# StractOrg/stract

Hardware: NVIDIA H100
Metric: webgraph_edges_per_sec_per_centrality_iter (higher is better)
Workload: dtype u8

## Files before the change

stract_b200/csrc/api_graph.cu:

```cuda
#include "graph.cuh"

#include <algorithm>
#include <vector>

namespace sb200 {
static thread_local char t_err[1024] = "";
std::atomic<uint64_t> g_launches{0};
thread_local cudaStream_t t_pool_stream = nullptr;
void set_error(const char* fmt, ...) {
  va_list ap; va_start(ap, fmt);
  vsnprintf(t_err, sizeof(t_err), fmt, ap);
  va_end(ap);
}
int hb_alloc_state(sb200_graph* g);
int hb_reset(sb200_graph* g);
int hb_step(sb200_graph* g, sb200_iter_stats* st);
int hb_step_launch(sb200_graph* g, bool with_barrier);
int hb_step_finish(sb200_graph* g, sb200_iter_stats* st);
int hb_barrier(sb200_graph* g);
__global__ void k_owned_flags(const uint32_t* __restrict__ inv, const uint32_t* __restrict__ sub, uint64_t N, uint32_t world, uint32_t rank,
                              uint8_t* owned, uint32_t* sub_out) {
  const uint64_t r = blockIdx.x * (uint64_t)blockDim.x + threadIdx.x;
  if (r >= N) return;
  const uint32_t v = inv[r];
  if (owned) owned[r] = (world <= 1 || ((v >> 5) % world) == rank) ? 1 : 0;
  if (sub_out) sub_out[r] = sub ? sub[v] : (world <= 1 ? 1u : 0xFFFFFFFFu >> (32 - world));
}
int hb_result(sb200_graph* g, uint64_t* id_lo, uint64_t* id_hi, double* cent, uint64_t cap, uint64_t* len);
int hb_registers(sb200_graph* g, uint64_t first, uint64_t count, uint8_t* out);
int hb_ranked(sb200_graph* g, int ties_desc, uint64_t* id_lo, uint64_t* id_hi, double* cent, uint64_t cap, uint64_t* len);
int hb_kahan(sb200_graph* g, uint64_t first, uint64_t count, double* sum, double* err);
}
using namespace sb200;

uint64_t sb200_graph::hbm_bytes() const {
  return id_lo.bytes() + id_hi.bytes() + perm.bytes() + inv.bytes() + row_ptr.bytes() + col.bytes() + fwd_ptr.bytes() +
         fwd_dst.bytes() + item_row.bytes() + item_start.bytes() + partial.bytes() + regs[0].bytes() + regs[1].bytes() +
         bm[0].bytes() + bm[1].bytes() + size_cache.bytes() + kahan_sum.bytes() + kahan_err.bytes() +
         frontier_list.bytes() + frontier_off.bytes() + cub_tmp.bytes() + counters.bytes() + sub_mask.bytes() + sync_page.bytes();
}

extern "C" {

const char* sb200_last_error(void) { return t_err; }
#ifndef SB200_EMU
const char* sb200_version(void) { return "stract_b200 0.1 (sm_90a)"; }
#else
const char* sb200_version(void) { return "stract_b200 0.1 CPU SIMT emulation (tests/emu, tests only)"; }
#endif
uint64_t sb200_kernel_launch_count(void) { return g_launches.load(); }

#define SB_ENTER(g)                                            \
  if (!(g)) SB_FAIL(SB200_EINVAL, "NULL graph handle");        \
  SB_CUDA(cudaSetDevice((g)->device))

int sb200_graph_create(const uint64_t* from_lo, const uint64_t* from_hi, const uint64_t* to_lo, const uint64_t* to_hi,
                       const uint64_t* rel_flags, uint64_t n_edges, uint64_t skipped_rel_mask, int device, int rank,
                       int world_size, sb200_graph** out) {
  if (!out) SB_FAIL(SB200_EINVAL, "out is NULL");
  *out = nullptr;
  if (world_size < 1 || world_size > 64 || rank < 0 || rank >= world_size)
    SB_FAIL(SB200_EINVAL, "bad rank/world_size %d/%d", rank, world_size);
  int ndev = 0;
  SB_CUDA(cudaGetDeviceCount(&ndev));
  if (device < 0 || device >= ndev) SB_FAIL(SB200_EINVAL, "device %d not in [0,%d)", device, ndev);
  SB_CUDA(cudaSetDevice(device));
  sb200_graph* g = new (std::nothrow) sb200_graph();
  if (!g) SB_FAIL(SB200_ENOMEM, "host allocation failed");
  g->device = device; g->rank = rank; g->world = world_size;
  int rc = SB200_OK;
  auto body = [&]() -> int {
    SB_CUDA(cudaStreamCreateWithFlags(&g->stream, cudaStreamNonBlocking));
    SB_CUDA(cudaEventCreate(&g->ev0)); SB_CUDA(cudaEventCreate(&g->ev1));
    SB_CUDA(cudaEventCreate(&g->ev_run0)); SB_CUDA(cudaEventCreate(&g->ev_run1));
    for (int f = 0; f < sb200_graph::F_COUNT; f++) { SB_CUDA(cudaEventCreate(&g->prof_ev[f][0])); SB_CUDA(cudaEventCreate(&g->prof_ev[f][1])); }
    {
      static bool pool_ready[64] = {false};
      if (device < 64 && !pool_ready[device]) {
        cudaMemPool_t pool; uint64_t keep = ~0ull;
        SB_CUDA(cudaDeviceGetDefaultMemPool(&pool, device));
        SB_CUDA(cudaMemPoolSetAttribute(pool, cudaMemPoolAttrReleaseThreshold, &keep));
        pool_ready[device] = true;
      }
      PoolScope scope(getenv("SB200_NO_POOL") ? nullptr : g->stream);
      SB_TRY(stage_graph(g, from_lo, from_hi, to_lo, to_hi, rel_flags, n_edges, skipped_rel_mask));
    }
    g->cub_tmp.release();
    {
      PoolScope scope((world_size == 1 && !getenv("SB200_NO_POOL")) ? g->stream : nullptr);
      SB_TRY(hb_alloc_state(g));
    }
    SB_TRY(hb_reset(g));
    return SB200_OK;
  };
  rc = body();
  if (rc != SB200_OK) { sb200_graph_destroy(g); return rc; }
  *out = g;
  return SB200_OK;
}

void sb200_graph_destroy(sb200_graph* g) {
  if (!g) return;
  cudaSetDevice(g->device);
  if (g->stream) cudaStreamSynchronize(g->stream);
  if (g->peers_ipc) for (int p = 0; p < g->n_peers; p++) for (int i = 0; i < 2; i++) {
    if (g->peer_regs[i][p]) cudaIpcCloseMemHandle(g->peer_regs[i][p]);
    if (g->peer_bm[i][p]) cudaIpcCloseMemHandle(g->peer_bm[i][p]);
  }
  if (g->peers_ipc) for (int p = 0; p < g->n_peers; p++) if (g->peer_sync[p]) cudaIpcCloseMemHandle(g->peer_sync[p]);
  if (g->l2_window_bytes) cudaCtxResetPersistingL2Cache();
  if (g->h_counters) cudaFreeHost(g->h_counters);
  if (g->ev0) cudaEventDestroy(g->ev0);
  if (g->ev1) cudaEventDestroy(g->ev1);
  if (g->side_stream) { cudaStreamSynchronize(g->side_stream); cudaStreamDestroy(g->side_stream); }
  if (g->ev_fork) cudaEventDestroy(g->ev_fork);
  if (g->ev_join) cudaEventDestroy(g->ev_join);
  for (int k = 0; k < 2; k++) if (g->side_prof[k]) cudaEventDestroy(g->side_prof[k]);
  if (g->ev_run0) cudaEventDestroy(g->ev_run0);
  if (g->ev_run1) cudaEventDestroy(g->ev_run1);
  for (int f = 0; f < sb200_graph::F_COUNT; f++) for (int k = 0; k < 2; k++) if (g->prof_ev[f][k]) cudaEventDestroy(g->prof_ev[f][k]);
  cudaStream_t s = g->stream;
  const int dev = g->device;
// ... 321 lines not shown
```

stract_b200/csrc/graph.cuh:

```cuda
#pragma once
#include "common.cuh"

namespace sb200 {
constexpr int MAX_PEERS = 15;
struct PeerOut { uint4* newr[MAX_PEERS]; uint32_t* bmc[MAX_PEERS]; const uint32_t* sub; int n; uint32_t world, rank; uint8_t prank[MAX_PEERS + 1]; };
constexpr int SYNC_SLOTS = 128;
struct SyncView { unsigned long long* local; unsigned long long* peer[MAX_PEERS]; int n; uint32_t world, rank; };
}

struct sb200_graph {
  int device = 0, rank = 0, world = 1;
  cudaStream_t stream = nullptr;
  cudaEvent_t ev0 = nullptr, ev1 = nullptr;
  uint64_t N = 0, E_in = 0, E_kept = 0, E_local = 0;
  uint64_t row_begin = 0, row_end = 0;
  uint64_t n_pos = 0;
  bool has_fwd = false;
  int reuse = 0;
  double stage_ms = 0;

  sb200::DevBuf<uint64_t> id_lo, id_hi;
  sb200::DevBuf<uint32_t> perm, inv;
  sb200::DevBuf<uint32_t> self_bm;
  sb200::DevBuf<uint32_t> row_ptr, col;
  uint32_t col_base = 0;
  sb200::DevBuf<uint32_t> fwd_ptr, fwd_dst;
  sb200::DevBuf<uint32_t> row_ranges_host_dummy;
  uint64_t range_begins[65] = {0};

  uint64_t warp_row_begin = 0, warp_row_end = 0;
  uint64_t quad_row_begin = 0, quad_row_end = 0;
  uint64_t n_items = 0;
  uint64_t n_multi_rows = 0;
  sb200::DevBuf<uint32_t> owned_items;
  uint64_t n_owned_items = 0;
  sb200::DevBuf<uint32_t> item_row, item_start;
  sb200::DevBuf<uint4> partial;
  uint64_t n_multi_items = 0;

  sb200::DevBuf<uint8_t> regs[2];
  sb200::DevBuf<uint32_t> bm[2];
  sb200::DevBuf<uint64_t> size_cache;
  sb200::DevBuf<double> kahan_sum, kahan_err;
  sb200::DevBuf<uint32_t> frontier_list, frontier_off;
  sb200::DevBuf<uint8_t> cub_tmp;
  sb200::DevBuf<unsigned long long> counters;
  unsigned long long* h_counters = nullptr;
  int cur = 0;
  int bcur = 0;
  uint32_t t = 0;
  bool has_changes = true;
  uint64_t n_changed_prev = 0, frontier_edges_prev = 0;
  bool exchange_pending = false;
  int n_peers = 0;
  bool p2p = false;
  bool peers_ipc = true;
  void* peer_regs[2][sb200::MAX_PEERS] = {{nullptr}};
  void* peer_bm[2][sb200::MAX_PEERS] = {{nullptr}};
  int peer_rank[sb200::MAX_PEERS] = {0};
  bool publish_all = false;
  sb200::DevBuf<uint32_t> sub_mask;
  uint64_t n_subscribed = 0;
  sb200::DevBuf<unsigned long long> sync_page;
  void* peer_sync[sb200::MAX_PEERS] = {nullptr};
  uint64_t sync_epoch = 0;
  bool step_in_flight = false, step_with_barrier = false;
  int step_mode = 0;
  double dense_frac = 0.35, push_div = 48.0;
  int force_mode = -1;
  uint64_t l2_window_bytes = 0;

  enum { F_PULL_WARP_DENSE, F_PULL_QUAD_DENSE, F_PULL_WARP_FRONT, F_PULL_QUAD_FRONT, F_PULL_MERGE, F_PUSH, F_FINALIZE, F_COUNT };
  bool profiling = false;
  uint64_t prof_launches[F_COUNT] = {0};
  double prof_ms[F_COUNT] = {0}, prof_bytes[F_COUNT] = {0};
  cudaEvent_t prof_ev[F_COUNT][2] = {{nullptr}};
  int sm_count = 0;
  int opt_side_ctas = -1, opt_owned_list = -1;
  cudaStream_t side_stream = nullptr;
  cudaEvent_t ev_fork = nullptr, ev_join = nullptr, side_prof[2] = {nullptr, nullptr};
  bool side_prof_used = false;
  int side_prof_family = 0;
  bool prof_used[F_COUNT] = {false};
  double prof_step_bytes[F_COUNT] = {0};
  uint64_t E_warp = 0, E_quad = 0;
  double own_frac = 1.0;
  cudaEvent_t ev_run0 = nullptr, ev_run1 = nullptr;
  float last_run_ms = 0;

  uint64_t hbm_bytes() const;
};

namespace sb200 {
constexpr int QUAD_MAX_DEG = 32;
constexpr int CHUNK_EDGES = 1024;

int build_fwd_csr(sb200_graph* g);
int stage_graph(sb200_graph* g, const uint64_t* from_lo, const uint64_t* from_hi, const uint64_t* to_lo,
                const uint64_t* to_hi, const uint64_t* rel, uint64_t n_edges, uint64_t mask);
}
```

stract_b200/csrc/hyperball.cu:

```cuda
#include <chrono>
#include "graph.cuh"
#include "../../include/sb200_hll_tables.h"

#ifndef SB200_EMU
#include <cub/cub.cuh>
#endif
#include <algorithm>
#include <cmath>
#include <cstdlib>

namespace sb200 {

struct HllTables {
  double raw[SB200_HLL_P5_LEN];
  double bias[SB200_HLL_P5_LEN];
  double lc[65];
};
__constant__ HllTables c_tab;
static bool g_tab_loaded[64] = {false};

int load_tables(int device) {
  if (device >= 0 && device < 64 && g_tab_loaded[device]) return SB200_OK;
  static HllTables h;
  for (int i = 0; i < SB200_HLL_P5_LEN; i++) { h.raw[i] = SB200_HLL_RAW_P5[i]; h.bias[i] = SB200_HLL_BIAS_P5[i]; }
// ... 218 lines not shown
  const unsigned ballA = __ballot_sync(0xffffffffu, ne_u4(accA, ownA)), ballB = __ballot_sync(0xffffffffu, ne_u4(accB, ownB));
  const bool chA = ((ballA >> (lane & ~3u)) & 0xFu) != 0u, chB = ((ballB >> (lane & ~3u)) & 0xFu) != 0u;
  if (liveA && (chA || bm_test(bm_prev, selfA))) newr[rowA * 4 + sub] = accA;
  if (liveA && chA && sub == 0) atomicOr(bm_cur + (selfA >> 5), 1u << (selfA & 31));
  if (liveB && (chB || bm_test(bm_prev, selfB))) newr[rowB * 4 + sub] = accB;
  if (liveB && chB && sub == 0) atomicOr(bm_cur + (selfB >> 5), 1u << (selfB & 31));
}

template <bool FRONTIER, bool LISTED>
__global__ void __launch_bounds__(256, 8) k_pull_warp(uint64_t n_items, uint64_t first_multi_free_item,
    const uint32_t* __restrict__ item_list, const uint32_t* __restrict__ item_row, const uint32_t* __restrict__ item_start, uint32_t warp_row_begin,
    const uint32_t* __restrict__ row_ptr, const uint32_t* __restrict__ col, uint32_t col_base,
    const uint4* __restrict__ oldr, uint4* __restrict__ newr, uint4* __restrict__ partial,
    const uint32_t* __restrict__ bm_prev, uint32_t* __restrict__ bm_cur, const PeerOut peers) {
  uint64_t item = (blockIdx.x * (uint64_t)blockDim.x + threadIdx.x) >> 5;
  if (item >= n_items) return;
  if (LISTED) item = item_list[item];
  const uint32_t lane = threadIdx.x & 31, sub = lane & 3, q = lane >> 2;
  const uint32_t row = item_row[item];
  if (!owned_row(peers, row)) return;
  const uint32_t chunk = (uint32_t)item - item_start[row - warp_row_begin];
  const uint32_t rs = row_ptr[row] - col_base, re = row_ptr[row + 1] - col_base;
  const uint32_t e0 = rs + chunk * (uint32_t)CHUNK_EDGES;
  const uint32_t e1 = min(e0 + (uint32_t)CHUNK_EDGES, re);
  uint4 acc = make_uint4(0, 0, 0, 0);
  uint32_t nxt = (e0 + lane < e1) ? ld_stream_u32(col + e0 + lane) : row;
  for (uint32_t base = e0; base < e1; base += 32) {
    uint32_t mine = nxt;
    nxt = (base + 32 + lane < e1) ? ld_stream_u32(col + base + 32 + lane) : row;
    if (FRONTIER) mine = bm_test(bm_prev, mine) ? mine : row;
    const uint32_t i0 = __shfl_sync(0xffffffffu, mine, q);
    const uint32_t i1 = __shfl_sync(0xffffffffu, mine, q + 8);
    const uint32_t i2 = __shfl_sync(0xffffffffu, mine, q + 16);
    const uint32_t i3 = __shfl_sync(0xffffffffu, mine, q + 24);
    const uint4 v0 = oldr[(uint64_t)i0 * 4 + sub];
    const uint4 v1 = oldr[(uint64_t)i1 * 4 + sub];
    const uint4 v2 = oldr[(uint64_t)i2 * 4 + sub];
    const uint4 v3 = oldr[(uint64_t)i3 * 4 + sub];
    acc = vmax_u8x16(vmax_u8x16(acc, v0), vmax_u8x16(vmax_u8x16(v1, v2), v3));
  }
#pragma unroll
  for (int off = 4; off < 32; off <<= 1) {
    uint4 o;
    o.x = __shfl_xor_sync(0xffffffffu, acc.x, off); o.y = __shfl_xor_sync(0xffffffffu, acc.y, off);
    o.z = __shfl_xor_sync(0xffffffffu, acc.z, off); o.w = __shfl_xor_sync(0xffffffffu, acc.w, off);
    acc = vmax_u8x16(acc, o);
  }
  if (item < first_multi_free_item) {
    if (q == 0) partial[item * 4 + sub] = acc;
    return;
  }
  const uint4 own = oldr[(uint64_t)row * 4 + sub];
  acc = vmax_u8x16(acc, own);
  const unsigned ball = __ballot_sync(0xffffffffu, ne_u4(acc, own));
  const bool changed = (ball & 0xFu) != 0u;
  if (q == 0) publish_row(newr, bm_cur, peers, row, sub, acc, changed || bm_test(bm_prev, row), changed);
}

__global__ void __launch_bounds__(256) k_pull_merge(uint64_t n_rows, const uint32_t* __restrict__ item_start,
    uint32_t warp_row_begin, const uint4* __restrict__ partial, const uint4* __restrict__ oldr,
    uint4* __restrict__ newr, const uint32_t* __restrict__ bm_prev, uint32_t* __restrict__ bm_cur, const PeerOut peers) {
  const uint64_t r = (blockIdx.x * (uint64_t)blockDim.x + threadIdx.x) >> 5;
  if (r >= n_rows) return;
  const uint32_t lane = threadIdx.x & 31, sub = lane & 3, q = lane >> 2;
  const uint32_t row = warp_row_begin + (uint32_t)r;
  if (!owned_row(peers, row)) return;
  const uint32_t i0 = item_start[r], i1 = item_start[r + 1];
  uint4 acc = make_uint4(0, 0, 0, 0);
  for (uint32_t it = i0 + q; it < i1; it += 8) acc = vmax_u8x16(acc, partial[(uint64_t)it * 4 + sub]);
#pragma unroll
  for (int off = 4; off < 32; off <<= 1) {
    uint4 o;
    o.x = __shfl_xor_sync(0xffffffffu, acc.x, off); o.y = __shfl_xor_sync(0xffffffffu, acc.y, off);
    o.z = __shfl_xor_sync(0xffffffffu, acc.z, off); o.w = __shfl_xor_sync(0xffffffffu, acc.w, off);
    acc = vmax_u8x16(acc, o);
  }
  const uint4 own = oldr[(uint64_t)row * 4 + sub];
  acc = vmax_u8x16(acc, own);
  const unsigned ball = __ballot_sync(0xffffffffu, ne_u4(acc, own));
  const bool changed = (ball & 0xFu) != 0u;
  if (q == 0) publish_row(newr, bm_cur, peers, row, sub, acc, changed || bm_test(bm_prev, row), changed);
}

__global__ void k_frontier_compact(const uint32_t* __restrict__ bm, uint64_t words, const uint32_t* __restrict__ fwd_ptr,
                                   uint32_t* list, uint32_t* outdeg, unsigned long long* counter,
                                   unsigned long long* slot_sum) {
  uint64_t w = blockIdx.x * (uint64_t)blockDim.x + threadIdx.x;
  if (w >= words) return;
  uint32_t m = bm[w];
  if (!m) return;
  unsigned long long pos = atomicAdd(counter, (unsigned long long)__popc(m));
  unsigned long long sum = 0;
  while (m) {
    int b = __ffs(m) - 1; m &= m - 1;
    uint32_t v = (uint32_t)(w * 32 + b);
    const uint32_t d = fwd_ptr[v + 1] - fwd_ptr[v];
    list[pos] = v; outdeg[pos] = d; pos++; sum += d;
  }
  if (slot_sum && sum) atomicAdd(slot_sum, sum);
}
__global__ void k_copy_stale(const uint32_t* __restrict__ list, uint64_t n, const uint4* __restrict__ oldr,
                             uint4* __restrict__ newr, uint32_t world, uint32_t rank) {
  uint64_t gt = blockIdx.x * (uint64_t)blockDim.x + threadIdx.x;
  uint64_t i = gt >> 2;
  if (i >= n) return;
  uint64_t v = list[i];
  if (world > 1 && ((v >> 5) % world) != rank) return;
  newr[v * 4 + (gt & 3)] = oldr[v * 4 + (gt & 3)];
}
__global__ void k_publish_rows(const uint32_t* __restrict__ bm_prev, const uint32_t* __restrict__ bm_cur, uint64_t n_rows,
                               const uint4* __restrict__ newr, const PeerOut peers) {
  const uint64_t gt = blockIdx.x * (uint64_t)blockDim.x + threadIdx.x;
  const uint64_t w = (gt >> 2) * peers.world + peers.rank;
  if (w * 32 >= n_rows) return;
  uint32_t m = __ldg(bm_prev + w) | __ldg(bm_cur + w);
  while (m) {
    const uint64_t row = w * 32 + (uint64_t)(__ffs(m) - 1);
    m &= m - 1;
    if (row >= n_rows) break;
    const uint4 v = newr[row * 4 + (gt & 3)];
    const uint32_t want = peers.sub ? __ldg(peers.sub + row) : 0xFFFFFFFFu;
    for (int p = 0; p < peers.n; p++) if ((want >> peers.prank[p]) & 1u) peers.newr[p][row * 4 + (gt & 3)] = v;
  }
}
__global__ void __launch_bounds__(256) k_push(const uint32_t* __restrict__ list, const uint32_t* __restrict__ off,
    uint32_t n_front, uint64_t n_slots, const uint32_t* __restrict__ fwd_ptr, const uint32_t* __restrict__ fwd_dst,
    const uint32_t* __restrict__ old32, uint32_t* new32, uint32_t* __restrict__ bm_cur) {
  const uint32_t lane = threadIdx.x & 31, l = lane & 15;
  const uint64_t hw = (blockIdx.x * (uint64_t)blockDim.x + threadIdx.x) >> 4;
  const uint64_t nhw = ((uint64_t)gridDim.x * blockDim.x) >> 4;
  for (uint64_t s = hw; s < ((n_slots + 1) & ~1ull); s += nhw) {
    bool changed = false;
    uint32_t v = 0;
    if (s < n_slots) {
      uint32_t lo = 0, hi = n_front;
      while (lo + 1 < hi) { uint32_t mid = (lo + hi) >> 1; if (off[mid] <= s) lo = mid; else hi = mid; }
      const uint32_t u = list[lo];
      v = fwd_dst[fwd_ptr[u] + (uint32_t)(s - off[lo])];
      const uint32_t mine = old32[(uint64_t)u * 16 + l];
      uint32_t* addr = new32 + (uint64_t)v * 16 + l;
      uint32_t cur = *addr;
      uint32_t m = bmax4_7bit(cur, mine);
      while (m != cur) {
        const uint32_t prev = atomicCAS(addr, cur, m);
        if (prev == cur) { changed = true; break; }
        cur = prev; m = bmax4_7bit(cur, mine);
      }
    }
    const unsigned ball = __ballot_sync(0xffffffffu, changed);
    const unsigned half = (lane < 16) ? (ball & 0xFFFFu) : (ball >> 16);
    if (half && l == 0) atomicOr(bm_cur + (v >> 5), 1u << (v & 31));
  }
}

__global__ void __launch_bounds__(256) k_finalize(uint64_t row_begin, uint64_t row_end,
    const uint4* __restrict__ newr, const uint32_t* __restrict__ bm_prev, const uint32_t* __restrict__ bm_cur,
    uint64_t* __restrict__ size_cache, double* __restrict__ ksum, double* __restrict__ kerr,
    const uint32_t* __restrict__ fwd_ptr, double t_plus_1, unsigned long long* counters, const uint32_t own_world,
    const uint32_t own_rank) {
  __shared__ HllTables tab;
  __shared__ unsigned long long s_cnt[2];
  for (int i = threadIdx.x; i < (int)(sizeof(HllTables) / 8); i += blockDim.x) ((double*)&tab)[i] = ((const double*)&c_tab)[i];
  if (threadIdx.x < 2) s_cnt[threadIdx.x] = 0;
  __syncthreads();
  const uint32_t lane = threadIdx.x & 31;
  const uint64_t world = own_world > 1 ? own_world : 1;
  const uint64_t warps = (uint64_t)gridDim.x * (blockDim.x >> 5), w0 = (uint64_t)blockIdx.x * (blockDim.x >> 5) + (threadIdx.x >> 5);
  const uint64_t b0 = row_begin >> 5, b1 = (row_end + 31) >> 5;
  const uint64_t first = b0 + ((uint64_t)own_rank + world - b0 % world) % world;
  unsigned long long my_changed = 0, my_out = 0;
  for (uint64_t b = first + w0 * world; b < b1; b += warps * world) {
    const uint32_t wc = __ldg(bm_cur + b), wp = __ldg(bm_prev + b);
    if ((wc | wp) == 0u) continue;
    const uint64_t v = b * 32 + lane;
    const bool bc = (wc >> lane) & 1u, bp = (wp >> lane) & 1u;
    if (v >= row_begin && v < row_end && (bc || bp)) {
      double s = ksum[v], e = kerr[v];
      if (bc) {
        uint32_t w[16];
#pragma unroll
        for (int q = 0; q < 4; q++) {
          const uint4 x = newr[v * 4 + q];
          w[4 * q] = x.x; w[4 * q + 1] = x.y; w[4 * q + 2] = x.z; w[4 * q + 3] = x.w;
        }
        const uint64_t sn = hll64_size(w, &tab);
        const uint64_t so = size_cache[v];
        const uint64_t d = sn >= so ? sn - so : 0ull;
        kahan_add(s, e, __ddiv_rn(__ull2double_rn(d), t_plus_1));
        size_cache[v] = sn;
        my_changed += 1;
        if (fwd_ptr) my_out += fwd_ptr[v + 1] - fwd_ptr[v];
      } else {
        kahan_add(s, e, 0.0);
      }
      ksum[v] = s; kerr[v] = e;
    }
  }
  for (int off = 16; off; off >>= 1) {
    my_changed += __shfl_down_sync(0xffffffffu, my_changed, off);
    my_out += __shfl_down_sync(0xffffffffu, my_out, off);
  }
  if ((threadIdx.x & 31) == 0 && (my_changed | my_out)) { atomicAdd(&s_cnt[0], my_changed); atomicAdd(&s_cnt[1], my_out); }
  __syncthreads();
  if (threadIdx.x == 0 && (s_cnt[0] | s_cnt[1])) { atomicAdd(counters + 0, s_cnt[0]); atomicAdd(counters + 1, s_cnt[1]); }
}

__global__ void k_result_flags(const uint32_t* __restrict__ inv, const double* __restrict__ ksum, uint64_t N,
                               uint64_t row_begin, uint64_t row_end, double norm, uint32_t* flag, double* val,
                               const uint32_t own_world, const uint32_t own_rank) {
  uint64_t r = blockIdx.x * (uint64_t)blockDim.x + threadIdx.x;
  if (r >= N) return;
  const uint32_t v = inv[r];
  double c = ksum[v];
  const bool keep = (c > 0.0) && v >= row_begin && v < row_end &&
                    (own_world <= 1 || ((v >> 5) % own_world) == own_rank);
  c = __ddiv_rn(c, norm);
  if (isinf(c) || isnan(c)) c = 0.0;
  flag[r] = keep ? 1u : 0u;
  val[r] = c;
}
__global__ void k_result_scatter(const uint32_t* __restrict__ flag, const uint32_t* __restrict__ pos,
                                 const double* __restrict__ val, const uint64_t* __restrict__ id_lo,
                                 const uint64_t* __restrict__ id_hi, uint64_t N, uint64_t cap, uint64_t* out_lo,
                                 uint64_t* out_hi, double* out_c) {
  uint64_t r = blockIdx.x * (uint64_t)blockDim.x + threadIdx.x;
  if (r >= N || !flag[r]) return;
  uint32_t p = pos[r];
  if (p >= cap) return;
  out_lo[p] = id_lo[r]; out_hi[p] = id_hi[r]; out_c[p] = val[r];
}
__global__ void k_gather_regs(const uint32_t* __restrict__ inv, const uint4* __restrict__ regs, uint64_t first,
                              uint64_t count, uint4* out) {
  uint64_t gt = blockIdx.x * (uint64_t)blockDim.x + threadIdx.x;
  uint64_t i = gt >> 2;
// ... 94 lines not shown
  }
  const int side_ctas = g->opt_side_ctas;
  const bool side_quad = side_ctas > 0 && g->world > 1 && g->p2p && g->n_peers > 0 && g->n_items && g->quad_row_end > g->quad_row_begin;
  if (side_quad) {
    if (!g->side_stream) {
      int lo = 0, hi = 0;
      SB_CUDA(cudaDeviceGetStreamPriorityRange(&lo, &hi));
      SB_CUDA(cudaStreamCreateWithPriority(&g->side_stream, cudaStreamNonBlocking, hi));
      SB_CUDA(cudaEventCreateWithFlags(&g->ev_fork, cudaEventDisableTiming));
      SB_CUDA(cudaEventCreateWithFlags(&g->ev_join, cudaEventDisableTiming));
      SB_CUDA(cudaEventCreate(&g->side_prof[0])); SB_CUDA(cudaEventCreate(&g->side_prof[1]));
    }
    if (!g->sm_count) SB_CUDA(cudaDeviceGetAttribute(&g->sm_count, cudaDevAttrMultiProcessorCount, g->device));
    const int sm_count = g->sm_count;
    const uint64_t world = (uint64_t)g->world, b0 = g->quad_row_begin >> 5, b1 = (g->quad_row_end - 1) >> 5;
    const uint64_t first = b0 + ((uint64_t)g->rank + world - b0 % world) % world;
    const uint64_t n_tasks = first <= b1 ? ((b1 - first) / world + 1) * 4 : 0;
    SB_CUDA(cudaEventRecord(g->ev_fork, s));
    SB_CUDA(cudaStreamWaitEvent(g->side_stream, g->ev_fork, 0));
    if (g->l2_window_bytes) {
      cudaStreamAttrValue a;
      memset(&a, 0, sizeof(a));
      a.accessPolicyWindow.base_ptr = (void*)oldr; a.accessPolicyWindow.num_bytes = g->l2_window_bytes;
      a.accessPolicyWindow.hitRatio = 1.0f; a.accessPolicyWindow.hitProp = cudaAccessPropertyPersisting;
      a.accessPolicyWindow.missProp = cudaAccessPropertyStreaming;
      SB_CUDA(cudaStreamSetAttribute(g->side_stream, cudaStreamAttributeAccessPolicyWindow, &a));
    }
    if (g->profiling) SB_CUDA(cudaEventRecord(g->side_prof[0], g->side_stream));
    if (getenv("SB200_DEBUG_SIDE")) fprintf(stderr, "[sb200] side quad: rank %d tasks %llu\n", g->rank, (unsigned long long)n_tasks);
    if (n_tasks) {
      const unsigned grid = (unsigned)std::min<uint64_t>(div_up(n_tasks, 8), (uint64_t)sm_count * (uint64_t)side_ctas);
      SB_LAUNCH(k_pull_quad_owned<FRONTIER>, grid, 256, 0, g->side_stream, g->quad_row_begin, g->quad_row_end, first, n_tasks,
                g->row_ptr.p, g->col.p, g->col_base, oldr, newr, bmp, bmc, po);
      SB_CHECK_LAUNCH();
    }
    if (g->profiling) {
      SB_CUDA(cudaEventRecord(g->side_prof[1], g->side_stream));
      g->side_prof_used = true; g->side_prof_family = FQ;
      g->prof_step_bytes[FQ] = g->own_frac * (per_edge * (double)g->E_quad + 68.0 * (double)(g->quad_row_end - g->quad_row_begin));
    }
  }
  if (g->n_items) {
    PROF_BEGIN(g, FW);
    if (g->opt_owned_list < 0) g->opt_owned_list = env_flag("SB200_OWNED_ITEMS", true) ? 1 : 0;
    const bool listed = g->opt_owned_list > 0 && g->world > 1 && g->owned_items.p;
    const uint64_t n_launch = listed ? g->n_owned_items : g->n_items;
    auto kern = listed ? k_pull_warp<FRONTIER, true> : k_pull_warp<FRONTIER, false>;
    if (n_launch)
    SB_LAUNCH(kern, div_up(n_launch * 32, 256), 256, 0, s, n_launch, g->n_multi_items,
              listed ? g->owned_items.p : (const uint32_t*)nullptr, g->item_row.p, g->item_start.p, (uint32_t)g->warp_row_begin, g->row_ptr.p, g->col.p, g->col_base, oldr, newr,
              g->partial.p, bmp, bmc, po);
    SB_CHECK_LAUNCH();
    PROF_END(g, FW, g->own_frac * (per_edge * (double)g->E_warp + 68.0 * (double)(g->warp_row_end - g->warp_row_begin - g->n_multi_rows)));
  }
  if (g->n_multi_rows) {
    PROF_BEGIN(g, sb200_graph::F_PULL_MERGE);
    SB_LAUNCH(k_pull_merge, div_up(g->n_multi_rows * 32, 256), 256, 0, s, g->n_multi_rows, g->item_start.p,
              (uint32_t)g->warp_row_begin, g->partial.p, oldr, newr, bmp, bmc, po);
    SB_CHECK_LAUNCH();
    PROF_END(g, sb200_graph::F_PULL_MERGE, 64.0 * (double)g->n_multi_items + 68.0 * (double)g->n_multi_rows);
  }
  const uint64_t nq = g->quad_row_end - g->quad_row_begin;
  if (side_quad) { SB_CUDA(cudaEventRecord(g->ev_join, g->side_stream)); SB_CUDA(cudaStreamWaitEvent(s, g->ev_join, 0)); }
  else if (nq) {
    PROF_BEGIN(g, FQ);
    static const bool quad2 = env_flag("SB200_QUAD2", false);
    if (quad2 && g->world == 1 && g->col_base == 0)
      SB_LAUNCH(k_pull_quad2<FRONTIER>, div_up(((nq + 1) / 2) * 4, 256), 256, 0, s, g->quad_row_begin, g->quad_row_end, g->row_ptr.p,
                g->col.p, oldr, newr, bmp, bmc);
    else
    SB_LAUNCH(k_pull_quad<FRONTIER>, div_up(nq * 4, 256), 256, 0, s, g->quad_row_begin, g->quad_row_end, g->row_ptr.p,
              g->col.p, g->col_base, oldr, newr, bmp, bmc, po);
    SB_CHECK_LAUNCH();
    PROF_END(g, FQ, g->own_frac * (per_edge * (double)g->E_quad + 68.0 * (double)nq));
  }
  return SB200_OK;
}

static int run_push(sb200_graph* g, const uint4* oldr, uint4* newr, const uint32_t* bmp, uint32_t* bmc) {
  cudaStream_t s = g->stream;
  const uint64_t N = g->N, words = (N + 31) / 32;
  const uint64_t nf = g->n_changed_prev;
  if (nf == 0) return SB200_OK;
  if (g->frontier_list.n < nf + 1) { SB_TRY(g->frontier_list.alloc(nf + 1 + (nf >> 2))); }
  if (g->frontier_off.n < 2 * (nf + 1)) { SB_TRY(g->frontier_off.alloc(2 * (nf + 1) + (nf >> 1))); }
  uint32_t* outdeg = g->frontier_off.p + (g->frontier_off.n / 2);
  SB_CUDA(cudaMemsetAsync(g->counters.p + 2, 0, 2 * sizeof(unsigned long long), s));
  SB_LAUNCH(k_frontier_compact, div_up(words, 256), 256, 0, s, bmp, words, g->fwd_ptr.p, g->frontier_list.p, outdeg,
            g->counters.p + 2, g->world > 1 ? g->counters.p + 3 : (unsigned long long*)nullptr);
  SB_CHECK_LAUNCH();
  uint64_t slots = g->frontier_edges_prev;
  if (g->world > 1) {
    unsigned long long h = 0;
    SB_CUDA(cudaMemcpyAsync(&h, g->counters.p + 3, sizeof(h), cudaMemcpyDeviceToHost, s));
    SB_CUDA(cudaStreamSynchronize(s));
    slots = h;
  }
  size_t need = 0;
  SB_CUDA(cub::DeviceScan::ExclusiveSum(nullptr, need, outdeg, g->frontier_off.p, (int64_t)nf, s));
  if (g->cub_tmp.n < need) SB_TRY(g->cub_tmp.alloc(need + 256));
  SB_CUDA(cub::DeviceScan::ExclusiveSum(g->cub_tmp.p, need, outdeg, g->frontier_off.p, (int64_t)nf, s));
  g_launches.fetch_add(2, std::memory_order_relaxed);
  SB_LAUNCH(k_copy_stale, div_up(nf * 4, 256), 256, 0, s, g->frontier_list.p, nf, oldr, newr, (uint32_t)g->world, (uint32_t)g->rank);
  SB_CHECK_LAUNCH();
  if (slots) {
    unsigned grid = (unsigned)std::min<uint64_t>(div_up(slots * 16, 256), 148u * 16u);
    PROF_BEGIN(g, sb200_graph::F_PUSH);
    SB_LAUNCH(k_push, grid, 256, 0, s, g->frontier_list.p, g->frontier_off.p, (uint32_t)nf, slots, g->fwd_ptr.p,
              g->fwd_dst.p, (const uint32_t*)oldr, (uint32_t*)newr, bmc);
    SB_CHECK_LAUNCH();
    PROF_END(g, sb200_graph::F_PUSH, 132.0 * (double)slots);
  }
  if (g->p2p && g->n_peers > 0) {
    const PeerOut po = make_peer_out(g, true);
    SB_LAUNCH(k_publish_rows, div_up(div_up(words, (uint64_t)g->world) * 4, 256), 256, 0, s, bmp, bmc, N, (const uint4*)newr, po);
    SB_CHECK_LAUNCH();
  }
  return SB200_OK;
}

__global__ void k_publish_bitmap(const uint32_t* __restrict__ bmc, uint64_t words, const PeerOut peers) {
  const uint64_t w = blockIdx.x * (uint64_t)blockDim.x + threadIdx.x;
  if (w >= words || (w % peers.world) != peers.rank) return;
  const uint32_t v = bmc[w];
  for (int p = 0; p < peers.n; p++) peers.bmc[p][w] = v;
}

__global__ void k_frontier_out_edges(const uint32_t* __restrict__ bm, uint64_t words, const uint32_t* __restrict__ fwd_ptr,
                                     unsigned long long* counter) {
  const uint64_t w = blockIdx.x * (uint64_t)blockDim.x + threadIdx.x;
  unsigned long long acc = 0;
  if (w < words) {
    uint32_t m = bm[w];
    while (m) { const int b = __ffs(m) - 1; m &= m - 1; const uint64_t v = w * 32 + b; acc += fwd_ptr[v + 1] - fwd_ptr[v]; }
  }
  for (int o = 16; o; o >>= 1) acc += __shfl_down_sync(0xffffffffu, acc, o);
  if ((threadIdx.x & 31) == 0 && acc) atomicAdd(counter, acc);
}

__device__ __forceinline__ void st_release_sys_u64(unsigned long long* p, unsigned long long v) {
#ifndef SB200_EMU
  asm volatile("st.release.sys.global.u64 [%0], %1;" :: "l"(p), "l"(v) : "memory");
#else
  *(volatile unsigned long long*)p = v;
#endif
}
__device__ __forceinline__ unsigned long long ld_acquire_sys_u64(const unsigned long long* p) {
#ifndef SB200_EMU
  unsigned long long v;
  asm volatile("ld.acquire.sys.global.u64 %0, [%1];" : "=l"(v) : "l"(p) : "memory");
  return v;
#else
  return *(const volatile unsigned long long*)p;
#endif
}
__device__ __forceinline__ unsigned long long global_ns() {
#ifndef SB200_EMU
  unsigned long long t;
  asm volatile("mov.u64 %0, %globaltimer;" : "=l"(t));
  return t;
#else
  return 0ull;
#endif
}
constexpr unsigned long long SYNC_COUNT_MASK = (1ull << 40) - 1;
__global__ void __launch_bounds__(32) k_barrier_count(const SyncView sv, unsigned long long epoch, const unsigned long long* __restrict__ count_in,
                                                      unsigned long long* out , unsigned long long timeout_ns) {
  const int lane = threadIdx.x;
  const unsigned long long e24 = epoch & 0xFFFFFFull;
  const unsigned long long cnt = count_in ? (*count_in & SYNC_COUNT_MASK) : 0ull;
  const unsigned long long val = (e24 << 40) | cnt;
  const uint32_t slot = (uint32_t)(epoch & 1ull) * 64u + sv.rank;
  __threadfence_system();
  if (lane < sv.n) st_release_sys_u64(sv.peer[lane] + slot, val);
  if (lane == sv.n) st_release_sys_u64(sv.local + slot, val);
  unsigned long long got = 0;
  bool ok = true;
  if (lane < (int)sv.world) {
    const unsigned long long* p = sv.local + (uint32_t)(epoch & 1ull) * 64u + lane;
    const unsigned long long t0 = global_ns();
    for (;;) {
      got = ld_acquire_sys_u64(p);
      if ((got >> 40) == e24) break;
      if (global_ns() - t0 > timeout_ns) { ok = false; got = 0; break; }
#ifdef SB200_EMU
      ok = false; got = 0; break;
#endif
    }
  }
  unsigned long long sum = (lane < (int)sv.world && ok) ? (got & SYNC_COUNT_MASK) : 0ull;
  for (int o = 16; o; o >>= 1) sum += __shfl_down_sync(0xffffffffu, sum, o);
  const unsigned bad = __ballot_sync(0xffffffffu, !ok);
// ... 287 lines not shown
```

Baseline: 75.57 billion.

## Deterministic frontier compaction via word scan and warp-tiled batched push kernel

```diff
diff --git a/stract_b200/csrc/api_graph.cu b/stract_b200/csrc/api_graph.cu
--- a/stract_b200/csrc/api_graph.cu
+++ b/stract_b200/csrc/api_graph.cu
@@ -37,7 +37,7 @@
   return id_lo.bytes() + id_hi.bytes() + perm.bytes() + inv.bytes() + row_ptr.bytes() + col.bytes() + fwd_ptr.bytes() +
          fwd_dst.bytes() + item_row.bytes() + item_start.bytes() + partial.bytes() + regs[0].bytes() + regs[1].bytes() +
          bm[0].bytes() + bm[1].bytes() + size_cache.bytes() + kahan_sum.bytes() + kahan_err.bytes() +
-         frontier_list.bytes() + frontier_off.bytes() + cub_tmp.bytes() + counters.bytes() + sub_mask.bytes() + sync_page.bytes();
+         frontier_list.bytes() + frontier_off.bytes() + frontier_scan.bytes() + cub_tmp.bytes() + counters.bytes() + sub_mask.bytes() + sync_page.bytes();
 }
 
 extern "C" {
diff --git a/stract_b200/csrc/graph.cuh b/stract_b200/csrc/graph.cuh
--- a/stract_b200/csrc/graph.cuh
+++ b/stract_b200/csrc/graph.cuh
@@ -43,6 +43,7 @@
   sb200::DevBuf<uint64_t> size_cache;
   sb200::DevBuf<double> kahan_sum, kahan_err;
   sb200::DevBuf<uint32_t> frontier_list, frontier_off;
+  sb200::DevBuf<unsigned long long> frontier_scan;
   sb200::DevBuf<uint8_t> cub_tmp;
   sb200::DevBuf<unsigned long long> counters;
   unsigned long long* h_counters = nullptr;
diff --git a/stract_b200/csrc/hyperball.cu b/stract_b200/csrc/hyperball.cu
--- a/stract_b200/csrc/hyperball.cu
+++ b/stract_b200/csrc/hyperball.cu
@@ -324,31 +324,53 @@
   if (q == 0) publish_row(newr, bm_cur, peers, row, sub, acc, changed || bm_test(bm_prev, row), changed);
 }
 
-__global__ void k_frontier_compact(const uint32_t* __restrict__ bm, uint64_t words, const uint32_t* __restrict__ fwd_ptr,
-                                   uint32_t* list, uint32_t* outdeg, unsigned long long* counter,
-                                   unsigned long long* slot_sum) {
-  uint64_t w = blockIdx.x * (uint64_t)blockDim.x + threadIdx.x;
+__global__ void k_frontier_count(const uint32_t* __restrict__ bm, uint64_t words, const uint32_t* __restrict__ fwd_ptr,
+                                 unsigned long long* __restrict__ word_sum) {
+  const uint64_t w = blockIdx.x * (uint64_t)blockDim.x + threadIdx.x;
+  if (w > words) return;
+  uint32_t m = w < words ? bm[w] : 0u;
+  uint32_t n = 0, d = 0;
+  while (m) {
+    const uint32_t v = (uint32_t)(w * 32 + (__ffs(m) - 1));
+    m &= m - 1;
+    const uint32_t dv = fwd_ptr[v + 1] - fwd_ptr[v];
+    n += dv != 0u; d += dv;
+  }
+  word_sum[w] = ((unsigned long long)n << 32) | d;
+}
+__global__ void k_frontier_scatter(const uint32_t* __restrict__ bm, uint64_t words, const uint32_t* __restrict__ fwd_ptr,
+                                   const unsigned long long* __restrict__ word_pos, uint32_t* __restrict__ list,
+                                   uint32_t* __restrict__ fbeg, uint32_t* __restrict__ off, unsigned long long* slot_total) {
+  const uint64_t w = blockIdx.x * (uint64_t)blockDim.x + threadIdx.x;
+  if (w > words) return;
+  const unsigned long long p = word_pos[w];
+  uint32_t j = (uint32_t)(p >> 32), o = (uint32_t)p;
+  if (w == words) {
+    off[j] = o;
+    if (slot_total) *slot_total = o;
+    return;
+  }
+  uint32_t m = bm[w];
+  while (m) {
+    const uint32_t v = (uint32_t)(w * 32 + (__ffs(m) - 1));
+    m &= m - 1;
+    const uint32_t f0 = fwd_ptr[v], dv = fwd_ptr[v + 1] - f0;
+    if (!dv) continue;
+    list[j] = v; fbeg[j] = f0; off[j] = o;
+    j++; o += dv;
+  }
+}
+__global__ void k_copy_stale(const uint32_t* __restrict__ bm, uint64_t words, const uint4* __restrict__ oldr,
+                             uint4* __restrict__ newr, uint32_t world, uint32_t rank) {
+  const uint64_t gt = blockIdx.x * (uint64_t)blockDim.x + threadIdx.x;
+  const uint64_t w = (gt >> 2) * world + rank;
   if (w >= words) return;
-  uint32_t m = bm[w];
-  if (!m) return;
-  unsigned long long pos = atomicAdd(counter, (unsigned long long)__popc(m));
-  unsigned long long sum = 0;
+  uint32_t m = __ldg(bm + w);
   while (m) {
-    int b = __ffs(m) - 1; m &= m - 1;
-    uint32_t v = (uint32_t)(w * 32 + b);
-    const uint32_t d = fwd_ptr[v + 1] - fwd_ptr[v];
-    list[pos] = v; outdeg[pos] = d; pos++; sum += d;
-  }
-  if (slot_sum && sum) atomicAdd(slot_sum, sum);
-}
-__global__ void k_copy_stale(const uint32_t* __restrict__ list, uint64_t n, const uint4* __restrict__ oldr,
-                             uint4* __restrict__ newr, uint32_t world, uint32_t rank) {
-  uint64_t gt = blockIdx.x * (uint64_t)blockDim.x + threadIdx.x;
-  uint64_t i = gt >> 2;
-  if (i >= n) return;
-  uint64_t v = list[i];
-  if (world > 1 && ((v >> 5) % world) != rank) return;
-  newr[v * 4 + (gt & 3)] = oldr[v * 4 + (gt & 3)];
+    const uint64_t v = w * 32 + (uint64_t)(__ffs(m) - 1);
+    m &= m - 1;
+    newr[v * 4 + (gt & 3)] = oldr[v * 4 + (gt & 3)];
+  }
 }
 __global__ void k_publish_rows(const uint32_t* __restrict__ bm_prev, const uint32_t* __restrict__ bm_cur, uint64_t n_rows,
                                const uint4* __restrict__ newr, const PeerOut peers) {
@@ -365,33 +387,74 @@
     for (int p = 0; p < peers.n; p++) if ((want >> peers.prank[p]) & 1u) peers.newr[p][row * 4 + (gt & 3)] = v;
   }
 }
-__global__ void __launch_bounds__(256) k_push(const uint32_t* __restrict__ list, const uint32_t* __restrict__ off,
-    uint32_t n_front, uint64_t n_slots, const uint32_t* __restrict__ fwd_ptr, const uint32_t* __restrict__ fwd_dst,
+constexpr int PUSH_BATCH = 4;
+constexpr int PUSH_CTAS_PER_SM = 6;
+__global__ void __launch_bounds__(256, PUSH_CTAS_PER_SM) k_push(const unsigned long long* __restrict__ total, const uint32_t* __restrict__ list,
+    const uint32_t* __restrict__ fbeg, const uint32_t* __restrict__ off, const uint32_t* __restrict__ fwd_dst,
     const uint32_t* __restrict__ old32, uint32_t* new32, uint32_t* __restrict__ bm_cur) {
-  const uint32_t lane = threadIdx.x & 31, l = lane & 15;
-  const uint64_t hw = (blockIdx.x * (uint64_t)blockDim.x + threadIdx.x) >> 4;
-  const uint64_t nhw = ((uint64_t)gridDim.x * blockDim.x) >> 4;
-  for (uint64_t s = hw; s < ((n_slots + 1) & ~1ull); s += nhw) {
-    bool changed = false;
-    uint32_t v = 0;
-    if (s < n_slots) {
-      uint32_t lo = 0, hi = n_front;
-      while (lo + 1 < hi) { uint32_t mid = (lo + hi) >> 1; if (off[mid] <= s) lo = mid; else hi = mid; }
-      const uint32_t u = list[lo];
-      v = fwd_dst[fwd_ptr[u] + (uint32_t)(s - off[lo])];
-      const uint32_t mine = old32[(uint64_t)u * 16 + l];
-      uint32_t* addr = new32 + (uint64_t)v * 16 + l;
-      uint32_t cur = *addr;
-      uint32_t m = bmax4_7bit(cur, mine);
-      while (m != cur) {
-        const uint32_t prev = atomicCAS(addr, cur, m);
-        if (prev == cur) { changed = true; break; }
-        cur = prev; m = bmax4_7bit(cur, mine);
+  const unsigned long long tot = *total;
+  const uint32_t n_src = (uint32_t)(tot >> 32), n_slots = (uint32_t)tot;
+  const uint32_t lane = threadIdx.x & 31, l = lane & 15, half = lane >> 4;
+  const uint64_t n_warps = ((uint64_t)gridDim.x * blockDim.x) >> 5;
+  const uint64_t warp = (blockIdx.x * (uint64_t)blockDim.x + threadIdx.x) >> 5;
+  const uint64_t tile = ((n_slots + n_warps - 1) / n_warps + 31) & ~31ull;
+  if (warp * tile >= n_slots) return;
+  const uint32_t s0 = (uint32_t)(warp * tile), s1 = (uint32_t)min(warp * tile + tile, (uint64_t)n_slots);
+  uint32_t lo = 0, hi = n_src;
+  while (lo + 1 < hi) { const uint32_t mid = (lo + hi) >> 1; if (off[mid] <= s0) lo = mid; else hi = mid; }
+  uint32_t cur = lo;
+  uint32_t row_u = 0xFFFFFFFFu, row = 0;
+  for (uint32_t S = s0; S < s1; S += 32) {
+    const uint32_t wj = min(cur + lane, n_src - 1);
+    const uint32_t w_end = off[min(cur + lane + 1, n_src)];
+    const uint32_t w_beg = off[wj], w_u = list[wj], w_f = fbeg[wj];
+    const uint32_t s = S + lane;
+    uint32_t k = 0;
+#pragma unroll
+    for (uint32_t step = 16; step; step >>= 1) {
+      const uint32_t e = __shfl_sync(0xffffffffu, w_end, k + step - 1);
+      if (e <= s) k += step;
+    }
+    const uint32_t u = __shfl_sync(0xffffffffu, w_u, k);
+    const uint32_t e_first = __shfl_sync(0xffffffffu, w_f, k) + (s - __shfl_sync(0xffffffffu, w_beg, k));
+    const uint32_t n_here = min(32u, s1 - S);
+    const uint32_t v = lane < n_here ? ld_stream_u32(fwd_dst + e_first) : 0u;
+    cur += __popc(__ballot_sync(0xffffffffu, w_end <= S + 32));
+    for (uint32_t p0 = 0; p0 < n_here; p0 += 2 * PUSH_BATCH) {
+      uint32_t dst[PUSH_BATCH], mine[PUSH_BATCH], old[PUSH_BATCH], want[PUSH_BATCH], got[PUSH_BATCH];
+      bool live[PUSH_BATCH];
+#pragma unroll
+      for (int q = 0; q < PUSH_BATCH; q++) {
+        const uint32_t from = p0 + 2 * q + half;
+        const uint32_t uq = __shfl_sync(0xffffffffu, u, from);
+        dst[q] = __shfl_sync(0xffffffffu, v, from);
+        live[q] = from < n_here;
+        if (live[q] && uq != row_u) { row = __ldg(old32 + (uint64_t)uq * 16 + l); row_u = uq; }
+        mine[q] = row;
       }
-    }
-    const unsigned ball = __ballot_sync(0xffffffffu, changed);
-    const unsigned half = (lane < 16) ? (ball & 0xFFFFu) : (ball >> 16);
-    if (half && l == 0) atomicOr(bm_cur + (v >> 5), 1u << (v & 31));
+#pragma unroll
+      for (int q = 0; q < PUSH_BATCH; q++) old[q] = live[q] ? new32[(uint64_t)dst[q] * 16 + l] : 0u;
+#pragma unroll
+      for (int q = 0; q < PUSH_BATCH; q++) {
+        want[q] = live[q] ? bmax4_7bit(old[q], mine[q]) : old[q];
+        got[q] = want[q] != old[q] ? atomicCAS(new32 + (uint64_t)dst[q] * 16 + l, old[q], want[q]) : old[q];
+      }
+#pragma unroll
+      for (int q = 0; q < PUSH_BATCH; q++) {
+        bool changed = want[q] != old[q] && got[q] == old[q];
+        if (want[q] != old[q] && !changed) {
+          uint32_t* addr = new32 + (uint64_t)dst[q] * 16 + l;
+          uint32_t c = got[q], m = bmax4_7bit(c, mine[q]);
+          while (m != c) {
+            const uint32_t prev = atomicCAS(addr, c, m);
+            if (prev == c) { changed = true; break; }
+            c = prev; m = bmax4_7bit(c, mine[q]);
+          }
+        }
+        const unsigned ball = __ballot_sync(0xffffffffu, changed);
+        if (((ball >> (16 * half)) & 0xFFFFu) && l == 0) atomicOr(bm_cur + (dst[q] >> 5), 1u << (dst[q] & 31));
+      }
+    }
   }
 }
 
@@ -652,12 +715,25 @@
   const uint64_t N = g->N, words = (N + 31) / 32;
   const uint64_t nf = g->n_changed_prev;
   if (nf == 0) return SB200_OK;
-  if (g->frontier_list.n < nf + 1) { SB_TRY(g->frontier_list.alloc(nf + 1 + (nf >> 2))); }
-  if (g->frontier_off.n < 2 * (nf + 1)) { SB_TRY(g->frontier_off.alloc(2 * (nf + 1) + (nf >> 1))); }
-  uint32_t* outdeg = g->frontier_off.p + (g->frontier_off.n / 2);
-  SB_CUDA(cudaMemsetAsync(g->counters.p + 2, 0, 2 * sizeof(unsigned long long), s));
-  SB_LAUNCH(k_frontier_compact, div_up(words, 256), 256, 0, s, bmp, words, g->fwd_ptr.p, g->frontier_list.p, outdeg,
-            g->counters.p + 2, g->world > 1 ? g->counters.p + 3 : (unsigned long long*)nullptr);
+  if (g->frontier_list.n < 2 * (nf + 1)) { SB_TRY(g->frontier_list.alloc(2 * (nf + 1) + (nf >> 1))); }
+  if (g->frontier_off.n < nf + 1) { SB_TRY(g->frontier_off.alloc(nf + 1 + (nf >> 2))); }
+  if (g->frontier_scan.n < 2 * (words + 1)) { SB_TRY(g->frontier_scan.alloc(2 * (words + 1))); }
+  uint32_t* list = g->frontier_list.p;
+  uint32_t* fbeg = g->frontier_list.p + g->frontier_list.n / 2;
+  unsigned long long* word_sum = g->frontier_scan.p;
+  unsigned long long* word_pos = g->frontier_scan.p + (words + 1);
+  SB_LAUNCH(k_frontier_count, div_up(words + 1, 256), 256, 0, s, bmp, words, g->fwd_ptr.p, word_sum);
+  SB_CHECK_LAUNCH();
+  size_t need = 0;
+  SB_CUDA(cub::DeviceScan::ExclusiveSum(nullptr, need, word_sum, word_pos, (int64_t)(words + 1), s));
+  if (g->cub_tmp.n < need) SB_TRY(g->cub_tmp.alloc(need + 256));
+  SB_CUDA(cub::DeviceScan::ExclusiveSum(g->cub_tmp.p, need, word_sum, word_pos, (int64_t)(words + 1), s));
+  g_launches.fetch_add(2, std::memory_order_relaxed);
+  SB_LAUNCH(k_frontier_scatter, div_up(words + 1, 256), 256, 0, s, bmp, words, g->fwd_ptr.p, word_pos, list, fbeg,
+            g->frontier_off.p, g->world > 1 ? g->counters.p + 3 : (unsigned long long*)nullptr);
+  SB_CHECK_LAUNCH();
+  SB_LAUNCH(k_copy_stale, div_up(div_up(words, (uint64_t)g->world) * 4, 256), 256, 0, s, bmp, words, oldr, newr,
+            (uint32_t)g->world, (uint32_t)g->rank);
   SB_CHECK_LAUNCH();
   uint64_t slots = g->frontier_edges_prev;
   if (g->world > 1) {
@@ -666,18 +742,12 @@
     SB_CUDA(cudaStreamSynchronize(s));
     slots = h;
   }
-  size_t need = 0;
-  SB_CUDA(cub::DeviceScan::ExclusiveSum(nullptr, need, outdeg, g->frontier_off.p, (int64_t)nf, s));
-  if (g->cub_tmp.n < need) SB_TRY(g->cub_tmp.alloc(need + 256));
-  SB_CUDA(cub::DeviceScan::ExclusiveSum(g->cub_tmp.p, need, outdeg, g->frontier_off.p, (int64_t)nf, s));
-  g_launches.fetch_add(2, std::memory_order_relaxed);
-  SB_LAUNCH(k_copy_stale, div_up(nf * 4, 256), 256, 0, s, g->frontier_list.p, nf, oldr, newr, (uint32_t)g->world, (uint32_t)g->rank);
-  SB_CHECK_LAUNCH();
   if (slots) {
-    unsigned grid = (unsigned)std::min<uint64_t>(div_up(slots * 16, 256), 148u * 16u);
+    if (!g->sm_count) SB_CUDA(cudaDeviceGetAttribute(&g->sm_count, cudaDevAttrMultiProcessorCount, g->device));
+    const unsigned grid = (unsigned)std::min<uint64_t>(div_up(slots, 32 * 8), (uint64_t)g->sm_count * PUSH_CTAS_PER_SM);
     PROF_BEGIN(g, sb200_graph::F_PUSH);
-    SB_LAUNCH(k_push, grid, 256, 0, s, g->frontier_list.p, g->frontier_off.p, (uint32_t)nf, slots, g->fwd_ptr.p,
-              g->fwd_dst.p, (const uint32_t*)oldr, (uint32_t*)newr, bmc);
+    SB_LAUNCH(k_push, grid, 256, 0, s, word_pos + words, list, fbeg, g->frontier_off.p, g->fwd_dst.p,
+              (const uint32_t*)oldr, (uint32_t*)newr, bmc);
     SB_CHECK_LAUNCH();
     PROF_END(g, sb200_graph::F_PUSH, 132.0 * (double)slots);
   }
```

Result: faster. 80.01 billion (median of 6 runs) (+5.9%).
